# metaphor/kfserving

Measured on AMD Instinct MI355X. Metric: predicted rows/sec (500-tree XGB, 28 feat), higher is better.
Workload: dtype f32; 1 GPU; C2 synthetic HIGGS-shaped XGBoost binary: 28 features, 500 trees depth 8, 1M-row batch per GPU; rows_per_gpu=1000000, trees=500, depth=8, features=28, layout=bheap, parallelism=rows sharded x1, x_buffers=3, streams=2

## Files before the change

### kfserving_amd/csrc/treeinfer.hip

```cpp
#include <hip/hip_runtime.h>

#include "treeinfer_forest.h"
#include "treeinfer_pack.h"
#include "treeinfer_shap.h"

namespace {

void free_scratch(DeviceForest& d) {
  if (d.x_buf) (void)hipFree(d.x_buf);
  if (d.out_buf) (void)hipFree(d.out_buf);
  if (d.hx_pin) (void)hipHostFree(d.hx_pin);
  if (d.ho_pin) (void)hipHostFree(d.ho_pin);
  for (int l = 0; l < 2; ++l) {
    if (d.lane_hx[l]) (void)hipHostFree(d.lane_hx[l]);
    if (d.lane_ho[l]) (void)hipHostFree(d.lane_ho[l]);
    if (d.lane_dx[l]) (void)hipFree(d.lane_dx[l]);
    if (d.lane_do[l]) (void)hipFree(d.lane_do[l]);
    if (d.lane_stream[l]) (void)hipStreamDestroy(d.lane_stream[l]);
  }
  static_cast<ScratchBufs&>(d) = ScratchBufs();
}

void free_device(DeviceForest& d) {
  if (d.device < 0) return;
// ... 187 lines not shown
  key = ti::KernelKey{};
  key.x64 = xdt == TI_F64;
  key.acc64 = f->accum == TI_F64;
  key.K = f->K;
  key.feat_lds = t.feat_lds;
  key.zero_rule = f->zero_rule != 0;

  KArgs& a = p->a;
  std::memset(&a, 0, sizeof(a));
  a.n_features = f->F;
  a.n_trees = f->T;
  a.n_groups = f->K;
  a.leaf_width = f->LW;
  a.kind = kind;
  a.transform = f->transform;
  a.base_first = f->base_first;
  a.lgb_zero_map = f->lgb_zero_map;
  a.divide = f->divisor != 1.0;
  a.transform_param = f->tparam;
  a.average_divisor = f->divisor;
  for (int k = 0; k < ti::kMaxGroups; ++k) a.base[k] = f->base[k];
  a.tree_group = d.tree_group;

  if (heap_fields(f->layout)) {
    const int64_t stride_b = xdt == TI_F64 ? f->stride64 : f->stride32;
    a.trees = xdt == TI_F64 ? d.heap64 : d.heap32;
    a.tree_stride = stride_b;
    a.heap_leaf_ids = d.heap_leaf_ids;
    a.depth = f->depth;
    const int64_t S = heap_stage_trees(f, xdt);
    if (S < 1) return fail(TI_ERR_UNSUPPORTED, "heap tree record does not fit in LDS");
    a.stage_trees = static_cast<int32_t>(S);
    p->lds += static_cast<size_t>(S * stride_b);
    key.walk = ti::Walk::Heap;
    if (f->layout == kLayoutCatHeap) {
      if (!t.feat_lds) return fail(TI_ERR_UNSUPPORTED, "categorical heap needs the LDS feature image");
      key.walk = f->has_cat_xgb != 0 ? ti::Walk::CatHeapXgb : ti::Walk::CatHeapLgb;
    }
  } else if (f->layout == kLayoutBinHeap) {
    const BinPlan& bi = f->bh[ii];
    const int64_t stride_b = bi.stride;
    const size_t fixed = align16(t.feat_bytes + 4);
    const size_t temp_min = 8 * static_cast<size_t>(R) * xs;
    auto area = [&](int64_t n) { return std::max(static_cast<size_t>(n * stride_b), temp_min); };
    const int64_t cap = static_cast<int64_t>(8) * 16 * R / stride_b;
    int64_t S = std::min<int64_t>(ti::kBTilp, cap);
    if (S < 1) return fail(TI_ERR_UNSUPPORTED, "binned heap tree record does not fit the stage");
    S = grow_stage(S, ti::kBTilp, cap, f->T, fixed, area);
    static const int force_s = env_int("TI_BHEAP_STAGE", 0);
    if (force_s > 0) S = std::min<int64_t>(force_s, cap);
    S = std::min<int64_t>(S, f->T);
    a.bin_mask = bi.mask;
    a.bin_kary = bi.kary;
    a.trees = d.bh_img[ii];
    a.tree_stride = stride_b;
    a.heap_leaf_ids = d.heap_leaf_ids;
    a.depth = f->depth;
    a.bin_tbl = d.bh_tbl[ii];
    a.bin_L = bi.L;
    a.bin_words = bi.words;
    key.bins16 = bi.b16 != 0;
    if (!bheap_fixed(f, xdt, kind)) {
      key.walk = ti::Walk::BinHeap;
      key.prefetch = S * stride_b <= static_cast<int64_t>(4) * 16 * R ? 4 : 8;
      const size_t ar = area(S);
      a.stage_trees = static_cast<int32_t>(S);
      a.stage_off = static_cast<int32_t>(fixed);
      a.bin_chunk = static_cast<int32_t>(std::min<size_t>((ar / (static_cast<size_t>(R) * xs)) & ~size_t(7),
                                                          static_cast<size_t>(f->F + 7) & ~size_t(7)));
      p->lds = fixed + ar;
    } else {
      const int ng = std::min(2, std::max(1, env_int("TI_BHEAP_NG", 1)));
      key.walk = ti::Walk::BinHeapFixed;
      key.groups = ng;
      a.stage_trees = 4 * ng;
      a.bin_chunk = 4 * ng;
      a.stage_off = static_cast<int32_t>(ti::kFixStage);
      if (d.bh_fix_img != nullptr) a.trees = d.bh_fix_img;
      p->lds = ti::kFixStage + static_cast<size_t>(4 * ng) * ti::kFixTree;
    }
  } else if (is_record(f->layout)) {
    const RecPlan& rx = f->rx[ii];
    a.rx_base = d.rx_base;
    a.rx_nint = d.rx_nint;
    a.leaf_base = d.leaf_base;
    a.leaves = d.leaves;
    a.exp_leaf_ids = d.exp_leaf_ids;
    a.bin_tbl = d.bx_tbl[ii];
    a.bin_L = rx.L;
    a.bin_kary = rx.kary;
    a.bin_words = rx.words;
    if (f->layout != kLayoutTopStaged) {
      a.rx_recs = d.rx_recs[ii];
      a.rx_slots = static_cast<uint32_t>(f->rx_slots);
    }
    if (has_heap_top(f->layout)) {
      a.trees = reinterpret_cast<const unsigned char*>(d.hx_top[ii]);
      a.depth = f->hx_top;
    }
    if (f->layout != kLayoutRecord) a.stage_off = static_cast<int32_t>(align16(t.feat_bytes + 4));
    if (stages_trees(f->layout)) {
      a.stage_start = d.lx_stage;
      a.n_stages = f->n_stages;
      p->lds = std::max(static_cast<size_t>(a.stage_off) + static_cast<size_t>(f->lx_stage_cap), kLxMinLds);
      if (p->lds > kLdsPerCu || static_cast<int64_t>(kLxPf) * 16 * R < f->lx_stage_cap)
        return fail(TI_ERR_UNSUPPORTED, f->layout == kLayoutStaged ? "staged record layout exceeds LDS"
                                                       : "heap-top staged layout exceeds LDS");
      a.bin_chunk = bin_chunk_for(static_cast<size_t>(f->lx_stage_cap), R, xdt, f->F);
    } else if (f->layout == kLayoutHeapTop) {
      a.tree_stride = static_cast<int64_t>(8) << f->hx_top;
      a.stage_trees = f->hx_stage;
      p->lds = static_cast<size_t>(a.stage_off) + static_cast<size_t>(f->hx_stage) * a.tree_stride;
      if (p->lds > kLdsPerCu || static_cast<int64_t>(kHxPf) * 16 * R < f->hx_stage * a.tree_stride)
        return fail(TI_ERR_UNSUPPORTED, "heap-top layout exceeds LDS");
      a.bin_chunk = bin_chunk_for(static_cast<size_t>(f->hx_stage) * a.tree_stride, R, xdt, f->F);
    }
    if (f->layout == kLayoutTopStaged) {
      a.tx_pos = d.tx8_pos;
      a.tx_vals = d.tx8_val;
      a.tx_ord = d.tx8_ord;
      a.bin_mask = f->tx16_mask;
      key.walk = f->tx8 == 3 ? ti::Walk::BottomU16Split : f->tx8 == 2 ? ti::Walk::BottomU16
                 : f->tx8 ? ti::Walk::BottomU8 : ti::Walk::HeapTopStaged;
      key.bins16 = rx.b8 == 0;
      if (f->tx8 == 3) p->block = 2 * R;
    } else {
      key.walk = f->layout == kLayoutRecord ? ti::Walk::Record
                 : f->layout == kLayoutStaged ? ti::Walk::StagedRecord : ti::Walk::HeapTopRecord;
    }
// ... 761 lines not shown
```

### kfserving_amd/csrc/treeinfer_forest.h

```cpp
#pragma once

#include <hip/hip_runtime.h>

#include <algorithm>
#include <atomic>
#include <chrono>
#include <cstdlib>
#include <cmath>
#include <limits>
#include <cstdio>
#include <cstring>
#include <memory>
#include <mutex>
#include <set>
#include <string>
#include <thread>
#include <utility>
#include <type_traits>
#include <vector>

#include "treeinfer.h"
#include "treeinfer_kernels.h"
#include "treeinfer_dispatch.h"
#include "treeinfer_linear.h"
// ... 158 lines not shown
  unsigned char* bh_tbl[2] = {nullptr, nullptr};
  unsigned char* bx_tbl[2] = {nullptr, nullptr};
  uint2* rx_recs[2] = {nullptr, nullptr};
  uint32_t* rx_base = nullptr;
  uint32_t* rx_nint = nullptr;
  int32_t* lx_stage = nullptr;
  uint32_t* tx8_pos = nullptr;
  void* tx8_val = nullptr;
  int32_t* tx8_ord = nullptr;
  uint32_t* hx_top[2] = {nullptr, nullptr};
  ti::LinLeaf* lin_leaves = nullptr;
  ti::LinTerm* lin_terms = nullptr;
  int64_t* lin_leaf_base = nullptr;
};

struct ShapPtrs {
  ShapPath* shap_paths = nullptr;
  ShapElem* shap_elems = nullptr;
  double* shap_leaf = nullptr;
  double* shap_bias = nullptr;
  void* shap_tab = nullptr;
  int64_t* shap_tab_off = nullptr;
};

struct ScratchBufs {
  void* x_buf = nullptr;
  size_t x_cap = 0;
  void* out_buf = nullptr;
  size_t out_cap = 0;
  void* hx_pin = nullptr;
  size_t hx_cap = 0;
  void* ho_pin = nullptr;
  size_t ho_cap = 0;
  hipStream_t lane_stream[2] = {nullptr, nullptr};
  void* lane_hx[2] = {nullptr, nullptr};
  void* lane_ho[2] = {nullptr, nullptr};
  void* lane_dx[2] = {nullptr, nullptr};
  void* lane_do[2] = {nullptr, nullptr};
  size_t lane_x_cap = 0, lane_o_cap = 0;
};

struct DeviceForest : ForestPtrs, ShapPtrs, ScratchBufs {
  int device = -1;
  hipStream_t stream = nullptr;
  DeviceAllocs forest_mem, shap_mem;
  std::atomic<int32_t> shap_tab_state{0};
  int64_t bytes = 0;
  std::mutex mu;
};

struct BinPlan {
  int32_t L = 0;
  int32_t kary = 0;
  int32_t b16 = 1;
  int32_t rows = 256;
  int32_t words = 0;
  int64_t stride = 0;
  uint32_t mask = ti::kBNodeOffMask;
};
struct BinImage : BinPlan {
  std::vector<unsigned char> img;
  std::vector<unsigned char> fix_img;
  std::vector<unsigned char> tbl;
};

struct RecPlan {
  int32_t L = 0;
  int32_t rows = 256;
  int32_t words = 0;
  int32_t kary = 0;
  int32_t b8 = 0;
};
struct RecExplicit : RecPlan {
  std::vector<uint2> recs;
  std::vector<unsigned char> tbl;
  std::vector<uint32_t> top;
};

struct RecArrays {
  RecExplicit rx[2];
  std::vector<int32_t> lx_stage;
  std::vector<uint32_t> tx_off, tx_nint;
  std::vector<uint32_t> tx8_pos;
  std::vector<unsigned char> tx8_val;
  std::vector<int32_t> tx8_ord;
};

struct HostImage {
  std::vector<int32_t> group;
  std::vector<unsigned char> heap32, heap64;
  std::vector<int32_t> heap_leaf_ids;
  BinImage bh[2];
  std::vector<ExpNode> nodes;
  std::vector<double> thr64;
  std::vector<int64_t> node_base, leaf_base;
  std::vector<int32_t> root, exp_leaf_ids;
  std::vector<uint32_t> cat_words;
  std::vector<unsigned char> leaves;
  std::vector<int64_t> exp_src;
  RecArrays rec;
  std::vector<uint32_t> rx_base, rx_nint;
  std::vector<ti::LinLeaf> lin_leaves;
  std::vector<ti::LinTerm> lin_terms;
  std::vector<int64_t> lin_leaf_base;
};

// ... 55 lines not shown
```

### kfserving_amd/csrc/treeinfer_kernels.h

```cpp
#pragma once

#include <hip/hip_runtime.h>
#include <stdint.h>

#include "treeinfer.h"

#ifndef TI_TILP
#define TI_TILP 8
#endif
#ifndef TI_ASM_STEP
#define TI_ASM_STEP 1
#endif
#ifndef TI_EXP_ILP
#define TI_EXP_ILP 4
#endif
#ifndef TI_BTILP
#define TI_BTILP 4
#endif
#ifndef TI_PF
#define TI_PF 8
#endif
#ifndef TI_BIN_Q
#define TI_BIN_Q 8
#endif
// ... 6 lines not shown
constexpr uint32_t kMetaCatXgb = 0x10000000u;
constexpr uint32_t kMetaFeatMask = 0x00FFFFFFu;
constexpr int kMaxGroups = 16;
constexpr int kExpIlp = TI_EXP_ILP;
constexpr int kTilp = TI_TILP;
constexpr int kBTilp = TI_BTILP;
constexpr int kPf = TI_PF;
typedef unsigned int u32x4 __attribute__((ext_vector_type(4)));

template <typename XT> struct HeapNode;
template <> struct HeapNode<float> { float thr; uint32_t meta; };
template <> struct HeapNode<double> { double thr; uint32_t meta; uint32_t pad; };

struct ExpNode { float thr; uint32_t meta; int32_t left; int32_t right; };

struct KArgs {
  const void* X;
  int64_t n_rows;
  int64_t row_stride;
  int32_t n_cols;
  int32_t n_features;
  int32_t n_trees;
  int32_t n_groups;
  int32_t leaf_width;
  int32_t kind;
  int32_t transform;
  int32_t base_first;
  int32_t lgb_zero_map;
  int32_t divide;
  int32_t depth;
  int32_t stage_trees;
  double transform_param;
  double average_divisor;
  double base[kMaxGroups];
  const unsigned char* trees;
  int64_t tree_stride;
  const int32_t* heap_leaf_ids;
  const ExpNode* nodes;
  const double* thr64;
  const int64_t* node_base;
  const int32_t* root;
  const int64_t* leaf_base;
  const void* leaves;
  const int32_t* exp_leaf_ids;
  const uint32_t* cat_words;
  const int32_t* stage_start;
  int32_t n_stages;
  const uint32_t* tx_pos;
  const void* tx_vals;
  const int32_t* tx_ord;
  const void* bin_tbl;
  int32_t bin_L;
  int32_t bin_kary;
  int32_t bin_words;
  int32_t bin_chunk;
  int32_t stage_off;
  uint32_t bin_mask;
  const uint2* rx_recs;
  const uint32_t* rx_base;
  const uint32_t* rx_nint;
  uint32_t rx_slots;
  const int32_t* tree_group;
  void* out;
};

__device__ __forceinline__ size_t align16(size_t x) { return (x + 15) & ~size_t(15); }

__device__ __forceinline__ float t_exp(float x) { return expf(x); }
__device__ __forceinline__ double t_exp(double x) { return exp(x); }
__device__ __forceinline__ float t_log1p(float x) { return log1pf(x); }
__device__ __forceinline__ double t_log1p(double x) { return log1p(x); }

template <typename XT>
__device__ __forceinline__ XT nan_value();
template <> __device__ __forceinline__ float nan_value<float>() { return __builtin_nanf(""); }
template <> __device__ __forceinline__ double nan_value<double>() { return __builtin_nan(""); }

template <typename XT>
__device__ __forceinline__ XT zero_map(XT v, int on) {
  return (on && __builtin_fabs((double)v) <= (double)1e-35f) ? XT(0) : v;
}

template <bool ZERO, bool CHECK_NAN = true, typename XT>
__device__ __forceinline__ bool go_left(XT x, XT thr, uint32_t meta) {
  bool left = x <= thr;
  if (CHECK_NAN) left = left || ((x != x) && (int32_t)meta < 0);
  if (ZERO) left = left != ((x == XT(0)) && (meta & kMetaZeroFlip) != 0);
  return left;
}

__device__ __forceinline__ bool cat_left(const uint32_t* bs, double x) {
  if (!(x > -1.0 && x < 2147483648.0)) return false;
  const uint32_t v = static_cast<uint32_t>(x);
  const uint32_t w = v >> 5;
  if (w >= bs[0]) return false;
  return (bs[1 + w] >> (v & 31u)) & 1u;
}

__device__ __forceinline__ bool cat_left_xgb(const uint32_t* bs, double x, uint32_t meta) {
  if (x != x) return (int32_t)meta < 0;
  if (!(x >= 0.0 && x < 16777216.0)) return true;
  const uint32_t v = static_cast<uint32_t>(x);
  const uint32_t w = v >> 5;
  if (w >= bs[0]) return true;
  return ((bs[1 + w] >> (v & 31u)) & 1u) == 0u;
}
// ... 249 lines not shown
  prefetch_stage(pf, reinterpret_cast<const u32x4*>(a.trees),
                 (int)(((int64_t)(T < S ? T : S) * stride) >> 4), tid, R);
  for (int t0 = 0; t0 < T; t0 += S) {
    const int cnt = (T - t0) < S ? (T - t0) : S;
    __syncthreads();
    commit_stage(pf, reinterpret_cast<u32x4*>(stage), (int)(((int64_t)cnt * stride) >> 4), tid, R);
    __syncthreads();
    {
      const int tn = t0 + S <= last0 ? t0 + S : last0;
      const int cn = (T - tn) < S ? (T - tn) : S;
      prefetch_stage(pf, reinterpret_cast<const u32x4*>(a.trees + (int64_t)tn * stride),
                     (int)(((int64_t)cn * stride) >> 4), tid, R);
    }
    if (tile_nan)
      heap_stage<XT, ACC, KMAX, FEAT_LDS, ZERO, true>(a, stage, cnt, t0, acc, lane_off, xrow, row, live);
    else
      heap_stage<XT, ACC, KMAX, FEAT_LDS, ZERO, false>(a, stage, cnt, t0, acc, lane_off, xrow, row, live);
  }
  if (!live || a.kind == TI_OUTPUT_LEAF) return;
  finish_row<ACC, KMAX>(acc, a, row);
}

constexpr uint32_t kBNodeNanLeft = 0x8000u;
constexpr uint32_t kBNodeOffMask = 0x7FFFu;
constexpr uint32_t kBNodeOffMask512 = 0x7803u;
constexpr uint32_t kBNodePairMask = 0x7F8u;

template <bool B16> struct BinTraits;
template <> struct BinTraits<true> { static constexpr int P = 2; static constexpr uint32_t kNan = 0xFFFFu; };
template <> struct BinTraits<false> { static constexpr int P = 4; static constexpr uint32_t kNan = 0xFFu; };

template <bool B16, bool CHECK_NAN>
__device__ __forceinline__ bool bin_left(uint32_t b, uint32_t nd) {
  bool left = b <= (nd >> 16);
  if (CHECK_NAN) left = left || (b == BinTraits<B16>::kNan && (nd & kBNodeNanLeft) != 0u);
  return left;
}

template <bool B16>
__device__ __forceinline__ uint32_t lds_bin(uint32_t byte_addr) {
  if (B16)
    return *reinterpret_cast<const __attribute__((address_space(3))) uint16_t*>(
        static_cast<uintptr_t>(byte_addr));
  return *reinterpret_cast<const __attribute__((address_space(3))) uint8_t*>(
      static_cast<uintptr_t>(byte_addr));
}

__device__ __forceinline__ uint32_t kpow5(int h) {
  uint32_t p = 1u;
  for (int i = 0; i < h; ++i) p *= 5u;
  return p;
}

template <typename XT, int Q>
__device__ __forceinline__ void rank_search(const KArgs& a, const XT (&x)[Q], int f0,
                                            uint32_t (&b)[Q]) {
  const int F = a.n_features;
  uint32_t tq[Q], k[Q];
  if (sizeof(XT) == 4 && a.bin_kary > 0) {
    typedef float f4_t __attribute__((ext_vector_type(4)));
    const f4_t* t4 = reinterpret_cast<const f4_t*>(a.bin_tbl);
    const uint32_t nn = (kpow5(a.bin_kary) - 1u) / 4u;
#pragma unroll
    for (int q = 0; q < Q; ++q) {
      tq[q] = (uint32_t)(f0 + q < F ? f0 + q : F - 1) * nn;
      k[q] = 0u;
    }
    for (int s = 0; s < a.bin_kary; ++s) {
      f4_t e[Q];
#pragma unroll
      for (int q = 0; q < Q; ++q) e[q] = t4[tq[q] + k[q]];
#pragma unroll
      for (int q = 0; q < Q; ++q) {
        const XT xv = x[q];
        const uint32_t c = (e[q].x < xv ? 1u : 0u) + (e[q].y < xv ? 1u : 0u) +
                           (e[q].z < xv ? 1u : 0u) + (e[q].w < xv ? 1u : 0u);
        k[q] = 5u * k[q] + 1u + c;
      }
    }
#pragma unroll
    for (int q = 0; q < Q; ++q) b[q] = 1u + k[q] - nn;
  } else {
    const XT* tbl = static_cast<const XT*>(a.bin_tbl);
    const uint32_t tsz = 1u << a.bin_L;
#pragma unroll
    for (int q = 0; q < Q; ++q) {
      tq[q] = (uint32_t)(f0 + q < F ? f0 + q : F - 1) * tsz;
      k[q] = 1u;
    }
    for (int s = 0; s < a.bin_L; ++s) {
      XT e[Q];
#pragma unroll
      for (int q = 0; q < Q; ++q) e[q] = tbl[tq[q] + k[q]];
#pragma unroll
      for (int q = 0; q < Q; ++q) k[q] = 2u * k[q] + (e[q] < x[q] ? 1u : 0u);
    }
#pragma unroll
    for (int q = 0; q < Q; ++q) b[q] = 1u + k[q] - tsz;
  }
}

template <typename XT, bool B16, int Q = TI_BIN_Q>
__device__ __forceinline__ bool stage_bins(volatile int* flag, XT* temp, const KArgs& a,
                                           int64_t row0, int R, int tid) {
  using BT = BinTraits<B16>;
  constexpr int P = BT::P;
  static_assert(Q % P == 0, "features searched at once: a multiple of the bins per word");
  const XT* X = static_cast<const XT*>(a.X);
  const int F = a.n_features;
  const int C = a.n_cols;
  const int64_t left_rows = a.n_rows - row0;
  const int rows_here = left_rows < R ? (int)left_rows : R;
  const bool vec_ok = ((reinterpret_cast<uintptr_t>(X) | (uintptr_t)(a.row_stride * sizeof(XT))) & 15) == 0;
  bool has_nan = false;
  if (tid == 0) *flag = 0;
  for (int f0 = 0; f0 < F; f0 += a.bin_chunk) {
    const int kc = (F - f0) < a.bin_chunk ? (F - f0) : a.bin_chunk;
    __syncthreads();
    constexpr int V = 16 / sizeof(XT);
    const bool vec = vec_ok && (f0 % V) == 0 && (kc % V) == 0 && f0 + kc <= C;
    const uint32_t n = (uint32_t)rows_here * (uint32_t)kc;
    const uint32_t ukc = (uint32_t)kc;
    if (vec) {
      typedef XT xv_t __attribute__((ext_vector_type(V)));
      const uint32_t kv = ukc / V;
      const uint32_t nv = (uint32_t)rows_here * kv;
      for (uint32_t e = tid; e < nv; e += R) {
        const uint32_t r = e / kv;
        const uint32_t cv = e - r * kv;
        const xv_t v = *reinterpret_cast<const xv_t*>(X + (row0 + r) * a.row_stride + f0 + cv * V);
#pragma unroll
        for (int j = 0; j < V; ++j) temp[(cv * V + j) * R + r] = zero_map(v[j], a.lgb_zero_map);
      }
    }
    for (uint32_t e = vec ? n : tid; e < n; e += R) {
      const uint32_t r = e / ukc;
      const uint32_t c = e - r * ukc;
      const int f = f0 + (int)c;
      const XT v = f < C ? X[(row0 + r) * a.row_stride + f] : nan_value<XT>();
      temp[c * R + r] = zero_map(v, a.lgb_zero_map);
    }
    __syncthreads();
    for (int c = 0; c < kc; c += Q) {
      XT x[Q];
#pragma unroll
      for (int q = 0; q < Q; ++q) x[q] = temp[(c + q < kc ? c + q : kc - 1) * R + tid];
      uint32_t b[Q];
      rank_search<XT, Q>(a, x, f0 + c, b);
      uint32_t w[Q / P];
#pragma unroll
      for (int j = 0; j < Q / P; ++j) w[j] = 0u;
#pragma unroll
      for (int q = 0; q < Q; ++q) {
        const bool nan = x[q] != x[q];
        has_nan |= nan && (c + q < kc);
        w[q / P] |= (nan ? BT::kNan : b[q]) << ((q % P) * (32 / P));
      }
#pragma unroll
      for (int j = 0; j < Q / P; ++j) {
        const int word = (f0 + c) / P + j;
        if (c + j * P < kc) {
          __attribute__((address_space(3))) uint32_t* dst =
              reinterpret_cast<__attribute__((address_space(3))) uint32_t*>(
                  static_cast<uintptr_t>((uint32_t)(word * R + tid) * 4u));
          *dst = w[j];
        }
      }
    }
  }
  if (has_nan && tid < rows_here) *flag = 1;
  __syncthreads();
  return *flag != 0;
}

template <typename ACC, int KMAX, bool B16, bool CHECK_NAN>
__device__ __forceinline__ void bheap_stage(const KArgs& a, const unsigned char* stage, int cnt,
                                            int t0, ACC (&acc)[KMAX], uint32_t lane_off,
                                            int64_t row, bool live) {
  const int D = a.depth;
  const int NE = 1 << D;
  const int T = a.n_trees;
  const int64_t stride = a.tree_stride;
  const bool want_leaf = a.kind == TI_OUTPUT_LEAF;
  for (int j = 0; j < cnt; j += kBTilp) {
    const uint32_t* tp[kBTilp];
    uint32_t idx[kBTilp], nd[kBTilp];
#pragma unroll
    for (int q = 0; q < kBTilp; ++q) {
      const int tq = (j + q) < cnt ? (j + q) : (cnt - 1);
      tp[q] = reinterpret_cast<const uint32_t*>(stage + (int64_t)tq * stride);
      idx[q] = 1u;
      nd[q] = tp[q][1];
    }
    for (int l = 0; l < D; ++l) {
      uint32_t b[kBTilp];
      uint2 pr[kBTilp];
#pragma unroll
      for (int q = 0; q < kBTilp; ++q) {
        b[q] = lds_bin<B16>((nd[q] & a.bin_mask) | lane_off);
        pr[q] = *reinterpret_cast<const uint2*>(tp[q] + 2u * idx[q]);
      }
#pragma unroll
      for (int q = 0; q < kBTilp; ++q) {
#if TI_ASM_STEP == 2
        if (!CHECK_NAN) {
          uint64_t m;
          asm("v_cmp_lt_u32_sdwa %2, %0, %3 src0_sel:WORD_1 src1_sel:DWORD\n\t"
              "v_cndmask_b32_e64 %0, %4, %5, %2\n\t"
              "v_addc_co_u32_e64 %1, %2, %1, %1, %2"
              : "+v"(nd[q]), "+v"(idx[q]), "=&s"(m) : "v"(b[q]), "v"(pr[q].x), "v"(pr[q].y));
          continue;
        }
#elif TI_ASM_STEP
        if (!CHECK_NAN) {
          asm("v_cmp_lt_u32_sdwa vcc, %0, %2 src0_sel:WORD_1 src1_sel:DWORD\n\t"
              "v_cndmask_b32 %0, %3, %4, vcc\n\t"
              "v_addc_co_u32 %1, vcc, %1, %1, vcc"
              : "+v"(nd[q]), "+v"(idx[q]) : "v"(b[q]), "v"(pr[q].x), "v"(pr[q].y)
              : "vcc");
          continue;
// ... 187 lines not shown
    constexpr int l_first = 1;
#else
    (void)top;
#pragma unroll
    for (int q = 0; q < 4; ++q) nd[q] = lds_u32(kFixStage + (uint32_t)((g * 4 + q) * kFixTree) + 4u);
    constexpr int l_first = 0;
#endif
#pragma unroll
    for (int l = l_first; l < 8; ++l) {
      uint32_t b[4];
      uint2 pr[4];
#pragma unroll
      for (int q = 0; q < 4; ++q) {
        b[q] = lds_bin<B16>((nd[q] & bmask) | lane_off);
        pr[q] = lds_u2c((nd[q] & kBNodePairMask) + (kFixStage + (uint32_t)((g * 4 + q) * kFixTree)));
      }
#pragma unroll
      for (int q = 0; q < 4; ++q) fix_step<B16, CHECK_NAN>(nd[q], b[q], pr[q]);
    }
#pragma unroll
    for (int q = 0; q < 4; ++q) {
      const int t = t0 + g * 4 + q;
      if (g * 4 + q < cnt) {
        const float v = __uint_as_float(nd[q]);
        add_leaf<float, KMAX>(acc, &v, 0, 1, KMAX == 1 ? 0 : a.tree_group[t]);
      }
    }
  }
}

template <typename XT, int KMAX, bool B16, int NG>
__global__ void __launch_bounds__(512) bheap_fix_kernel(const KArgs a) {
  extern __shared__ __attribute__((aligned(16))) unsigned char smem[];
  constexpr int R = kFixRows;
  constexpr int S = 4 * NG;
  const int tid = threadIdx.x;
  const int64_t row0 = (int64_t)blockIdx.x * R;
  const int64_t row = row0 + tid;
  const bool live = row < a.n_rows;
  volatile int* flag = reinterpret_cast<volatile int*>(smem + kFixFlag);
  u32x4* stage = reinterpret_cast<u32x4*>(smem + kFixStage);
  const uint32_t lane_off = (uint32_t)tid * 4u;
  const int T = a.n_trees;
  constexpr int n16 = S * kFixTree / 16;
  static_assert(n16 == NG * R, "one 16-byte word per thread and group");
  const u32x4* src = reinterpret_cast<const u32x4*>(a.trees);
  const int n16_all = (int)(((int64_t)T * kFixTree) >> 4);
  u32x4 pf[NG];
#pragma unroll
  for (int u = 0; u < NG; ++u) {
    const int i = tid + u * R;
    pf[u] = src[i < n16_all ? i : n16_all - 1];
  }
  const bool tile_nan = stage_bins<XT, B16, 4 * NG>(
      flag, reinterpret_cast<XT*>(smem + kFixStage), a, row0, R, tid);
  float acc[KMAX];
  init_acc(acc, a);
  u32x4 top[4 * NG] = {};
  for (int t0 = 0; t0 < T; t0 += S) {
    const int cnt = (T - t0) < S ? (T - t0) : S;
    __syncthreads();
#if TI_FIX_SROOT
    fix_tops<NG>(a, t0, top);
#endif
#pragma unroll
    for (int u = 0; u < NG; ++u) stage[tid + u * R] = pf[u];
    __syncthreads();
    {
      const int base = (t0 + S) * (kFixTree / 16);
#pragma unroll
      for (int u = 0; u < NG; ++u) {
        const int i = base + tid + u * R;
        pf[u] = src[i < n16_all ? i : n16_all - 1];
      }
    }
    if (tile_nan)
      bheap_fix_stage<KMAX, B16, true, NG>(a, cnt, t0, acc, lane_off, top);
    else
      bheap_fix_stage<KMAX, B16, false, NG>(a, cnt, t0, acc, lane_off, top);
  }
  if (!live) return;
  finish_row<float, KMAX>(acc, a, row);
}

template <typename XT, typename ACC, int KMAX, bool FEAT_LDS, bool ZERO>
__global__ void __launch_bounds__(512) explicit_predict_kernel(const KArgs a) {
  extern __shared__ __attribute__((aligned(16))) unsigned char smem[];
  const int R = blockDim.x;
  const int tid = threadIdx.x;
  const int64_t row0 = (int64_t)blockIdx.x * R;
  const int64_t row = row0 + tid;
  const bool live = row < a.n_rows;
  XT* feat = reinterpret_cast<XT*>(smem);
  const XT* xrow = static_cast<const XT*>(a.X) + (live ? row : a.n_rows - 1) * a.row_stride;
  if (FEAT_LDS) {
    volatile int* flag = reinterpret_cast<volatile int*>(
        smem + align16((size_t)a.n_features * R * sizeof(XT)));
    stage_features<XT>(feat, flag, a, row0, R, tid);
  }
  const int T = a.n_trees;
  const bool want_leaf = a.kind == TI_OUTPUT_LEAF;
  int32_t* out_leaf = static_cast<int32_t*>(a.out);
  const ACC* leaves = static_cast<const ACC*>(a.leaves);

  ACC acc[KMAX];
  init_acc(acc, a);

// ... 1201 lines not shown
```

### kfserving_amd/csrc/treeinfer_pack.h

```cpp
#pragma once

#include "treeinfer_forest.h"

namespace {

int validate(const ti_forest_desc* d, std::vector<int>* depth_out) {
  if (!d) return fail(TI_ERR_INVALID, "null forest descriptor");
  if (d->abi_version != TI_ABI_VERSION)
    return fail(TI_ERR_INVALID, "abi_version mismatch: got " + std::to_string(d->abi_version));
  if (d->n_trees <= 0) return fail(TI_ERR_INVALID, "n_trees must be > 0");
  if (d->n_features <= 0 || d->n_features > (1 << 24))
    return fail(TI_ERR_INVALID, "n_features out of range");
  if (d->n_groups <= 0) return fail(TI_ERR_INVALID, "n_groups must be > 0");
  if (d->n_groups > (1 << 20)) return fail(TI_ERR_UNSUPPORTED, "n_groups > 2^20");
  if (d->leaf_width != 1 && d->leaf_width != d->n_groups)
    return fail(TI_ERR_INVALID, "leaf_width must be 1 or n_groups");
  if (d->accum_dtype != TI_F32 && d->accum_dtype != TI_F64)
    return fail(TI_ERR_INVALID, "accum_dtype must be TI_F32 or TI_F64");
  if (d->transform < TI_TRANSFORM_IDENTITY || d->transform > TI_TRANSFORM_STEP)
    return fail(TI_ERR_INVALID, "unknown transform");
  if (!(d->average_divisor > 0.0)) return fail(TI_ERR_INVALID, "average_divisor must be > 0");
  if (!d->tree_offset || !d->feature || !d->threshold || !d->flags || !d->left || !d->right ||
      !d->leaf_id || !d->leaf_value || !d->base_margin)
    return fail(TI_ERR_INVALID, "null array in forest descriptor");
// ... 356 lines not shown
  return rt;
}

template <typename XT>
void eytzinger_tables(const RankTables<XT>& rt, std::vector<unsigned char>* out) {
  const int F = static_cast<int>(rt.u.size());
  const size_t tsz = static_cast<size_t>(1) << rt.L;
  out->assign(static_cast<size_t>(F) * tsz * sizeof(XT), 0);
  XT* tbl = reinterpret_cast<XT*>(out->data());
  std::vector<double> srt, ey(tsz);
  for (int f = 0; f < F; ++f) {
    srt.assign(rt.u[f].begin(), rt.u[f].end());
    size_t i = 0;
    std::fill(ey.begin(), ey.end(), static_cast<double>(INFINITY));
    eytzinger_fill(srt, &ey, 1, &i);
    for (size_t k = 0; k < tsz; ++k) tbl[f * tsz + k] = static_cast<XT>(ey[k]);
  }
}

template <typename XT>
void kary_fill(const std::vector<XT>& srt, std::vector<XT>* out, size_t j, int level, int H,
               size_t* i) {
  if (level == H) return;
  for (int c = 0; c < 4; ++c) {
    kary_fill(srt, out, 5 * j + 1 + c, level + 1, H, i);
    (*out)[4 * j + c] = *i < srt.size() ? srt[*i] : static_cast<XT>(INFINITY);
    ++*i;
  }
  kary_fill(srt, out, 5 * j + 5, level + 1, H, i);
}

template <typename XT>
void kary_tables(const RankTables<XT>& rt, std::vector<unsigned char>* out, int* height) {
  const int F = static_cast<int>(rt.u.size());
  int H = 1;
  size_t p5 = 5;
  while (p5 - 1 < rt.m_max) {
    p5 *= 5;
    ++H;
  }
  const size_t nn = (p5 - 1) / 4;
  out->assign(static_cast<size_t>(F) * nn * 4 * sizeof(XT), 0);
  std::vector<XT> node(nn * 4), srt;
  for (int f = 0; f < F; ++f) {
    srt.assign(rt.u[f].begin(), rt.u[f].end());
    size_t i = 0;
    kary_fill(srt, &node, 0, 0, H, &i);
    std::memcpy(out->data() + static_cast<size_t>(f) * nn * 4 * sizeof(XT), node.data(),
                nn * 4 * sizeof(XT));
  }
  *height = H;
}

void fix_permute(BinImage* bi, const std::vector<double>& hcov, int NE) {
  const int64_t T = static_cast<int64_t>(bi->img.size()) / bi->stride;
  bi->fix_img.assign(bi->img.size(), 0);
  std::vector<int32_t> pi(NE, 0), lvl;
  for (int64_t t = 0; t < T; ++t) {
    const uint32_t* on = reinterpret_cast<const uint32_t*>(bi->img.data() + bi->stride * t);
    const float* ol = reinterpret_cast<const float*>(on + NE);
    uint32_t* nn = reinterpret_cast<uint32_t*>(bi->fix_img.data() + bi->stride * t);
    float* nl = reinterpret_cast<float*>(nn + NE);
    const double* c = hcov.data() + static_cast<size_t>(t) * NE;
    for (int lo = 1; lo < NE; lo <<= 1) {
      lvl.resize(lo);
      for (int i = 0; i < lo; ++i) lvl[i] = lo + i;
      std::stable_sort(lvl.begin(), lvl.end(), [c](int32_t x, int32_t y) { return c[x] > c[y]; });
      for (int i = 0; i < lo; ++i) pi[lvl[i]] = lo + i;
    }
    auto relabel = [&](uint32_t w, int h) { return (w & ~0x7F8u) | (static_cast<uint32_t>(pi[h]) << 3); };
    nn[1] = relabel(on[1], 1);
    for (int v = 1; v < NE; ++v)
      for (int s = 0; s < 2; ++s) {
        const int ch = 2 * v + s, nw = 2 * pi[v] + s;
        if (ch < NE) nn[nw] = relabel(on[ch], ch);
        else nl[nw - NE] = ol[ch - NE];
      }
  }
}

template <typename XT, typename ACC>
bool pack_bheap(const ti_forest_desc* d, int D, BinImage* out,
                std::vector<int32_t>* leaf_ids) {
  const int F = d->n_features;
  const int LW = d->leaf_width;
  const RankTables<XT> rt = collect_ranks<XT>(d, false);
  const size_t m_max = rt.m_max;
  if (m_max > 65533) return false;
  BinImage image;
  BinImage* const bi = &image;
  bi->b16 = m_max > 253 ? 1 : 0;
  const int P = bi->b16 ? 2 : 4;
  bi->words = (F + P - 1) / P;
  int R = 64;
  while (R < 512 && 2 * R <= env_int("TI_BHEAP_ROWS", 512)) R *= 2;
  while (R > 64 && static_cast<int64_t>(bi->words) * R * 4 > static_cast<int64_t>(ti::kBNodeOffMask) + 1)
    R >>= 1;
  if (static_cast<int64_t>(bi->words) * R * 4 > static_cast<int64_t>(ti::kBNodeOffMask) + 1) return false;
  bi->rows = R;
  bi->L = rt.L;
  bi->kary = 0;
  if constexpr (sizeof(XT) == 4) {
    if (env_int("TI_KARY", 1) != 0) kary_tables(rt, &bi->tbl, &bi->kary);
    else eytzinger_tables(rt, &bi->tbl);
  } else {
    eytzinger_tables(rt, &bi->tbl);
  }
  const bool with_index = R == 512;
  bi->mask = with_index ? ti::kBNodeOffMask512 : ti::kBNodeOffMask;
  auto node_word = [&](int64_t g) -> uint32_t {
    const int f = d->feature[g];
    const uint32_t rank = rt.rank(f, d->threshold[g]);
    const uint32_t off = static_cast<uint32_t>((f / P) * R * 4 + (f % P) * (4 / P));
    uint32_t w = off | (rank << 16);
    if (d->flags[g] & TI_NODE_NAN_LEFT) w |= ti::kBNodeNanLeft;
    return w;
  };
  const int NE = 1 << D;
  bi->stride = static_cast<int64_t>(align16(sizeof(uint32_t) * NE + sizeof(ACC) * NE * LW));
  bi->img.assign(static_cast<size_t>(bi->stride) * d->n_trees, 0);
  if (leaf_ids) leaf_ids->assign(static_cast<size_t>(NE) * d->n_trees, 0);
  struct Item { int32_t node; int32_t heap; int32_t level; double cov; };
  std::vector<Item> st;
  const bool perm = sizeof(XT) == 4 && sizeof(ACC) == 4 && with_index && D == 8 && LW == 1 && d->cover &&
                    env_int("TI_FIX_PERM", 1) != 0;
  std::vector<double> hcov(perm ? static_cast<size_t>(NE) * d->n_trees : 0, 0.0);
  for (int t = 0; t < d->n_trees; ++t) {
    unsigned char* rec = bi->img.data() + static_cast<size_t>(bi->stride) * t;
    uint32_t* nodes = reinterpret_cast<uint32_t*>(rec);
    ACC* leaves = reinterpret_cast<ACC*>(rec + sizeof(uint32_t) * NE);
    const int64_t b = d->tree_offset[t];
    st.assign(1, Item{0, 1, 0, d->cover ? d->cover[b] : 0.0});
    while (!st.empty()) {
      const Item it = st.back();
      st.pop_back();
      const int64_t g = b + it.node;
      if (perm && it.level < D) hcov[static_cast<size_t>(t) * NE + it.heap] = it.cov;
      if (it.level == D) {
        const int slot = it.heap - NE;
        for (int k = 0; k < LW; ++k)
          leaves[static_cast<size_t>(slot) * LW + k] = static_cast<ACC>(d->leaf_value[g * LW + k]);
        if (leaf_ids) (*leaf_ids)[static_cast<size_t>(t) * NE + slot] = d->leaf_id[g];
        continue;
      }
      const uint32_t idx = with_index ? static_cast<uint32_t>(it.heap) << 3 : 0u;
      if (d->feature[g] < 0) {
        nodes[it.heap] = (0xFFFFu << 16) | idx;
        st.push_back(Item{it.node, 2 * it.heap, it.level + 1, it.cov});
        st.push_back(Item{it.node, 2 * it.heap + 1, it.level + 1, 0.0});
      } else {
        nodes[it.heap] = node_word(g) | idx;
        st.push_back(Item{d->left[g], 2 * it.heap, it.level + 1,
                          d->cover ? d->cover[b + d->left[g]] : 0.0});
        st.push_back(Item{d->right[g], 2 * it.heap + 1, it.level + 1,
                          d->cover ? d->cover[b + d->right[g]] : 0.0});
      }
    }
  }
  if (perm) fix_permute(bi, hcov, NE);
  *out = std::move(image);
  return true;
}

struct RecSlots {
  std::vector<uint32_t> slot_of;
  std::vector<uint32_t> rx_base, rx_nint;
  int64_t rx_slots = 0;
};
struct RecCandidate : RecArrays {
  int64_t lx_stage_cap = 0;
  int32_t lx_ilp = 8;
  int32_t hx_top = 0, hx_stage = 0, hx_ilp = 8;
  int32_t tx8 = 0;
  uint32_t tx16_mask = 0;
};

bool plan_rx_slots(const ti_forest_desc* d, RecSlots* out) {
  std::vector<int32_t> level, next;
  RecSlots s;
  std::vector<uint32_t>* const slot_of = &s.slot_of;
  slot_of->assign(d->n_nodes, 0);
  s.rx_base.assign(d->n_trees + 1, 0);
  s.rx_nint.assign(d->n_trees, 0);
  if (d->n_nodes >= (int64_t(1) << 31)) return false;
  std::vector<int32_t> q;
  for (int t = 0; t < d->n_trees; ++t) {
    const int64_t b = d->tree_offset[t];
    const int64_t n = d->tree_offset[t + 1] - b;
    if (n > 65535) return false;
    s.rx_base[t] = static_cast<uint32_t>(b);
    level.assign(1, 0);
    uint32_t n_int = 0;
    while (!level.empty()) {
      cover_order(d, b, &level);
      next.clear();
      for (const int32_t v : level) {
        const int64_t g = b + v;
        if (d->feature[g] < 0) continue;
        (*slot_of)[g] = n_int++;
        next.push_back(d->left[g]);
        next.push_back(d->right[g]);
      }
      level.swap(next);
    }
    leaf_order(d, b, &q);
    for (size_t i = 0; i < q.size(); ++i) (*slot_of)[b + q[i]] = n_int + static_cast<uint32_t>(i);
    s.rx_nint[t] = n_int;
  }
  s.rx_base[d->n_trees] = static_cast<uint32_t>(d->n_nodes);
  s.rx_slots = d->n_nodes;
  *out = std::move(s);
  return true;
// ... 671 lines not shown
```

Before: 1.798 billion rows/s.

## Add bucketed threshold lookup, register-prefetched binning, and LDS bank-spread node permutation

Replaces the k-ary threshold search used to bin float features with a uniform bucket index table. Each feature value maps arithmetically to a bucket, which points into the sorted thresholds, so only four comparisons are needed. It adds a register-prefetch path for the fixed binned-heap kernel that loads the next 16-byte feature vector from global memory while the current chunk is binned. Separately, the heap node permutation now spreads hot nodes across 32 LDS bank classes by cover. Together these target binning cost and bank conflicts during traversal, in exchange for a larger table and extra build-time logic.

Result: faster. 1.850 billion rows/s (median of 6 runs) (+2.8%).

```diff
diff --git a/kfserving_amd/csrc/treeinfer.hip b/kfserving_amd/csrc/treeinfer.hip
--- a/kfserving_amd/csrc/treeinfer.hip
+++ b/kfserving_amd/csrc/treeinfer.hip
@@ -263,6 +263,7 @@
     S = std::min<int64_t>(S, f->T);
     a.bin_mask = bi.mask;
     a.bin_kary = bi.kary;
+    a.bin_nb = bi.bkt_nb;
     a.trees = d.bh_img[ii];
     a.tree_stride = stride_b;
     a.heap_leaf_ids = d.heap_leaf_ids;
@@ -286,6 +287,7 @@
       key.groups = ng;
       a.stage_trees = 4 * ng;
       a.bin_chunk = 4 * ng;
+      a.bin_xpf = env_int("TI_BIN_XPF", 1) != 0;
       a.stage_off = static_cast<int32_t>(ti::kFixStage);
       if (d.bh_fix_img != nullptr) a.trees = d.bh_fix_img;
       p->lds = ti::kFixStage + static_cast<size_t>(4 * ng) * ti::kFixTree;
diff --git a/kfserving_amd/csrc/treeinfer_forest.h b/kfserving_amd/csrc/treeinfer_forest.h
--- a/kfserving_amd/csrc/treeinfer_forest.h
+++ b/kfserving_amd/csrc/treeinfer_forest.h
@@ -234,6 +234,7 @@
 struct BinPlan {
   int32_t L = 0;
   int32_t kary = 0;
+  int32_t bkt_nb = 0;
   int32_t b16 = 1;
   int32_t rows = 256;
   int32_t words = 0;
diff --git a/kfserving_amd/csrc/treeinfer_kernels.h b/kfserving_amd/csrc/treeinfer_kernels.h
--- a/kfserving_amd/csrc/treeinfer_kernels.h
+++ b/kfserving_amd/csrc/treeinfer_kernels.h
@@ -82,6 +82,8 @@
   const void* bin_tbl;
   int32_t bin_L;
   int32_t bin_kary;
+  int32_t bin_nb;
+  int32_t bin_xpf;
   int32_t bin_words;
   int32_t bin_chunk;
   int32_t stage_off;
@@ -437,12 +439,48 @@
   return p;
 }
 
+__host__ __device__ __forceinline__ uint32_t bin_bucket(float x, float lo, float scale, int32_t nb) {
+#ifdef __HIP_DEVICE_COMPILE__
+  float t = __fmul_rn(__fsub_rn(x, lo), scale);
+#else
+  volatile float d = x - lo;
+  float t = d * scale;
+#endif
+  t = fminf(fmaxf(t, 0.0f), static_cast<float>(nb - 1));
+  int32_t k = static_cast<int32_t>(t);
+  k = k < 0 ? 0 : k;
+  k = k > nb - 1 ? nb - 1 : k;
+  return static_cast<uint32_t>(k);
+}
+
 template <typename XT, int Q>
 __device__ __forceinline__ void rank_search(const KArgs& a, const XT (&x)[Q], int f0,
                                             uint32_t (&b)[Q]) {
   const int F = a.n_features;
   uint32_t tq[Q], k[Q];
-  if (sizeof(XT) == 4 && a.bin_kary > 0) {
+  if (sizeof(XT) == 4 && a.bin_nb > 0) {
+    const uint32_t nb = (uint32_t)a.bin_nb;
+    const uint4* fs = reinterpret_cast<const uint4*>(a.bin_tbl);
+    const uint16_t* start = reinterpret_cast<const uint16_t*>(fs + F);
+    const float* srt = reinterpret_cast<const float*>(start + (size_t)F * nb);
+    typedef float f4u_t __attribute__((ext_vector_type(4), aligned(4)));
+#pragma unroll
+    for (int q = 0; q < Q; ++q) {
+      const uint32_t f = (uint32_t)(f0 + q < F ? f0 + q : F - 1);
+      const uint4 p = fs[f];
+      k[q] = start[f * nb + bin_bucket((float)x[q], __uint_as_float(p.x), __uint_as_float(p.y), a.bin_nb)];
+      tq[q] = p.z + k[q];
+    }
+    f4u_t e[Q];
+#pragma unroll
+    for (int q = 0; q < Q; ++q) e[q] = *reinterpret_cast<const f4u_t*>(srt + tq[q]);
+#pragma unroll
+    for (int q = 0; q < Q; ++q) {
+      const float xv = (float)x[q];
+      b[q] = 1u + k[q] + (e[q].x < xv ? 1u : 0u) + (e[q].y < xv ? 1u : 0u) + (e[q].z < xv ? 1u : 0u) +
+             (e[q].w < xv ? 1u : 0u);
+    }
+  } else if (sizeof(XT) == 4 && a.bin_kary > 0) {
     typedef float f4_t __attribute__((ext_vector_type(4)));
     const f4_t* t4 = reinterpret_cast<const f4_t*>(a.bin_tbl);
     const uint32_t nn = (kpow5(a.bin_kary) - 1u) / 4u;
@@ -485,7 +523,37 @@
   }
 }
 
-template <typename XT, bool B16, int Q = TI_BIN_Q>
+template <typename XT, bool B16, int Q>
+__device__ __forceinline__ bool bin_commit(const KArgs& a, const XT (&x)[Q], int f, int n, int R,
+                                           int tid) {
+  using BT = BinTraits<B16>;
+  constexpr int P = BT::P;
+  uint32_t b[Q];
+  rank_search<XT, Q>(a, x, f, b);
+  uint32_t w[Q / P];
+  bool has_nan = false;
+#pragma unroll
+  for (int j = 0; j < Q / P; ++j) w[j] = 0u;
+#pragma unroll
+  for (int q = 0; q < Q; ++q) {
+    const bool nan = x[q] != x[q];
+    has_nan |= nan && (q < n);
+    w[q / P] |= (nan ? BT::kNan : b[q]) << ((q % P) * (32 / P));
+  }
+#pragma unroll
+  for (int j = 0; j < Q / P; ++j) {
+    const int word = f / P + j;
+    if (j * P < n) {
+      __attribute__((address_space(3))) uint32_t* dst =
+          reinterpret_cast<__attribute__((address_space(3))) uint32_t*>(
+              static_cast<uintptr_t>((uint32_t)(word * R + tid) * 4u));
+      *dst = w[j];
+    }
+  }
+  return has_nan;
+}
+
+template <typename XT, bool B16, int Q = TI_BIN_Q, bool REGS = false>
 __device__ __forceinline__ bool stage_bins(volatile int* flag, XT* temp, const KArgs& a,
                                            int64_t row0, int R, int tid) {
   using BT = BinTraits<B16>;
@@ -499,10 +567,28 @@
   const bool vec_ok = ((reinterpret_cast<uintptr_t>(X) | (uintptr_t)(a.row_stride * sizeof(XT))) & 15) == 0;
   bool has_nan = false;
   if (tid == 0) *flag = 0;
+  constexpr int V = 16 / sizeof(XT);
+  if constexpr (Q == V && REGS) {
+    if (a.bin_xpf != 0 && vec_ok && a.bin_chunk == V && F % V == 0 && F <= C) {
+      typedef XT xv_t __attribute__((ext_vector_type(V)));
+      const XT* xr = X + (row0 + (tid < rows_here ? tid : 0)) * a.row_stride;
+      xv_t nx = *reinterpret_cast<const xv_t*>(xr);
+      __syncthreads();
+      for (int f0 = 0; f0 < F; f0 += V) {
+        XT x[Q];
+#pragma unroll
+        for (int q = 0; q < Q; ++q) x[q] = zero_map(nx[q], a.lgb_zero_map);
+        if (f0 + V < F) nx = *reinterpret_cast<const xv_t*>(xr + f0 + V);
+        has_nan |= bin_commit<XT, B16, Q>(a, x, f0, V, R, tid);
+      }
+      if (has_nan && tid < rows_here) *flag = 1;
+      __syncthreads();
+      return *flag != 0;
+    }
+  }
   for (int f0 = 0; f0 < F; f0 += a.bin_chunk) {
     const int kc = (F - f0) < a.bin_chunk ? (F - f0) : a.bin_chunk;
     __syncthreads();
-    constexpr int V = 16 / sizeof(XT);
     const bool vec = vec_ok && (f0 % V) == 0 && (kc % V) == 0 && f0 + kc <= C;
     const uint32_t n = (uint32_t)rows_here * (uint32_t)kc;
     const uint32_t ukc = (uint32_t)kc;
@@ -530,27 +616,7 @@
       XT x[Q];
 #pragma unroll
       for (int q = 0; q < Q; ++q) x[q] = temp[(c + q < kc ? c + q : kc - 1) * R + tid];
-      uint32_t b[Q];
-      rank_search<XT, Q>(a, x, f0 + c, b);
-      uint32_t w[Q / P];
-#pragma unroll
-      for (int j = 0; j < Q / P; ++j) w[j] = 0u;
-#pragma unroll
-      for (int q = 0; q < Q; ++q) {
-        const bool nan = x[q] != x[q];
-        has_nan |= nan && (c + q < kc);
-        w[q / P] |= (nan ? BT::kNan : b[q]) << ((q % P) * (32 / P));
-      }
-#pragma unroll
-      for (int j = 0; j < Q / P; ++j) {
-        const int word = (f0 + c) / P + j;
-        if (c + j * P < kc) {
-          __attribute__((address_space(3))) uint32_t* dst =
-              reinterpret_cast<__attribute__((address_space(3))) uint32_t*>(
-                  static_cast<uintptr_t>((uint32_t)(word * R + tid) * 4u));
-          *dst = w[j];
-        }
-      }
+      has_nan |= bin_commit<XT, B16, Q>(a, x, f0 + c, kc - c, R, tid);
     }
   }
   if (has_nan && tid < rows_here) *flag = 1;
@@ -844,7 +910,7 @@
     const int i = tid + u * R;
     pf[u] = src[i < n16_all ? i : n16_all - 1];
   }
-  const bool tile_nan = stage_bins<XT, B16, 4 * NG>(
+  const bool tile_nan = stage_bins<XT, B16, 4 * NG, (KMAX <= 4)>(
       flag, reinterpret_cast<XT*>(smem + kFixStage), a, row0, R, tid);
   float acc[KMAX];
   init_acc(acc, a);
diff --git a/kfserving_amd/csrc/treeinfer_pack.h b/kfserving_amd/csrc/treeinfer_pack.h
--- a/kfserving_amd/csrc/treeinfer_pack.h
+++ b/kfserving_amd/csrc/treeinfer_pack.h
@@ -432,7 +432,67 @@
   *height = H;
 }
 
-void fix_permute(BinImage* bi, const std::vector<double>& hcov, int NE) {
+int bucket_starts(const RankTables<float>& rt, int NB, std::vector<float>* ls,
+                  std::vector<uint16_t>* start) {
+  const int F = static_cast<int>(rt.u.size());
+  ls->assign(static_cast<size_t>(F) * 2, 0.0f);
+  start->assign(static_cast<size_t>(F) * NB, 0);
+  std::vector<size_t> cnt;
+  size_t occ_max = 0;
+  for (int f = 0; f < F; ++f) {
+    const std::vector<float>& u = rt.u[f];
+    float lo = 0.0f, scale = 0.0f;
+    if (!u.empty()) lo = u.front();
+    if (u.size() > 1) {
+      const float span = u.back() - lo;
+      scale = static_cast<float>(NB) / span;
+      if (!std::isfinite(span) || !std::isfinite(scale) || !(scale > 0.0f)) return -1;
+    }
+    (*ls)[2 * f] = lo;
+    (*ls)[2 * f + 1] = scale;
+    cnt.assign(NB, 0);
+    for (float t : u) ++cnt[ti::bin_bucket(t, lo, scale, NB)];
+    size_t below = 0;
+    for (int k = 0; k < NB; ++k) {
+      (*start)[static_cast<size_t>(f) * NB + k] = static_cast<uint16_t>(below);
+      below += cnt[k];
+      occ_max = std::max(occ_max, cnt[k]);
+    }
+  }
+  return static_cast<int>(occ_max);
+}
+
+bool bucket_tables(const RankTables<float>& rt, std::vector<unsigned char>* out, int* nb_out) {
+  const int F = static_cast<int>(rt.u.size());
+  if (rt.m_max <= 24) return false;
+  int NB = 2;
+  while (NB < 4096 && static_cast<size_t>(NB) < rt.m_max) NB *= 2;
+  std::vector<float> ls;
+  std::vector<uint16_t> start;
+  int occ = bucket_starts(rt, NB, &ls, &start);
+  while (occ > 4 && NB < 4096) occ = bucket_starts(rt, NB *= 2, &ls, &start);
+  if (occ < 0 || occ > 4) return false;
+  struct Feat { float lo, scale; uint32_t first, pad; };
+  size_t keys = 0;
+  for (int f = 0; f < F; ++f) keys += rt.u[f].size() + 4;
+  const size_t b_fs = static_cast<size_t>(F) * sizeof(Feat), b_st = start.size() * sizeof(uint16_t);
+  out->assign(b_fs + b_st + keys * sizeof(float), 0);
+  Feat* fs = reinterpret_cast<Feat*>(out->data());
+  std::memcpy(out->data() + b_fs, start.data(), b_st);
+  float* srt = reinterpret_cast<float*>(out->data() + b_fs + b_st);
+  size_t at = 0;
+  for (int f = 0; f < F; ++f) {
+    fs[f] = Feat{ls[2 * f], ls[2 * f + 1], static_cast<uint32_t>(at), 0u};
+    at = std::copy(rt.u[f].begin(), rt.u[f].end(), srt + at) - srt;
+    std::fill(srt + at, srt + at + 4, INFINITY);
+    at += 4;
+  }
+  *nb_out = NB;
+  return true;
+}
+
+void fix_permute(BinImage* bi, const std::vector<double>& hcov, int NE, bool spread) {
+  constexpr int kCls = 32;
   const int64_t T = static_cast<int64_t>(bi->img.size()) / bi->stride;
   bi->fix_img.assign(bi->img.size(), 0);
   std::vector<int32_t> pi(NE, 0), lvl;
@@ -446,7 +506,20 @@
       lvl.resize(lo);
       for (int i = 0; i < lo; ++i) lvl[i] = lo + i;
       std::stable_sort(lvl.begin(), lvl.end(), [c](int32_t x, int32_t y) { return c[x] > c[y]; });
-      for (int i = 0; i < lo; ++i) pi[lvl[i]] = lo + i;
+      if (!spread || lo <= kCls) {
+        for (int i = 0; i < lo; ++i) pi[lvl[i]] = lo + i;
+        continue;
+      }
+      double load[kCls] = {0};
+      int used[kCls] = {0};
+      for (int i = 0; i < lo; ++i) {
+        int k = -1;
+        for (int b = 0; b < kCls; ++b)
+          if (used[b] < lo / kCls && (k < 0 || load[b] < load[k])) k = b;
+        pi[lvl[i]] = lo + k + kCls * used[k];
+        load[k] += c[lvl[i]];
+        ++used[k];
+      }
     }
     auto relabel = [&](uint32_t w, int h) { return (w & ~0x7F8u) | (static_cast<uint32_t>(pi[h]) << 3); };
     nn[1] = relabel(on[1], 1);
@@ -481,8 +554,11 @@
   bi->L = rt.L;
   bi->kary = 0;
   if constexpr (sizeof(XT) == 4) {
-    if (env_int("TI_KARY", 1) != 0) kary_tables(rt, &bi->tbl, &bi->kary);
-    else eytzinger_tables(rt, &bi->tbl);
+    const bool kary = env_int("TI_KARY", 1) != 0;
+    const bool bkt = kary && env_int("TI_BIN_BUCKETS", 1) != 0 &&
+                     bucket_tables(rt, &bi->tbl, &bi->bkt_nb);
+    if (!bkt && kary) kary_tables(rt, &bi->tbl, &bi->kary);
+    if (!bkt && !kary) eytzinger_tables(rt, &bi->tbl);
   } else {
     eytzinger_tables(rt, &bi->tbl);
   }
@@ -537,7 +613,7 @@
       }
     }
   }
-  if (perm) fix_permute(bi, hcov, NE);
+  if (perm) fix_permute(bi, hcov, NE, env_int("TI_FIX_SPREAD", 1) != 0);
   *out = std::move(image);
   return true;
 }
```
